# HsinyuG/mobile-manipulator-mpc

Hardware: AMD Instinct MI355X
Metric: MPC solves/sec, whole-body N=20 batch=8192 (higher is better)
Workload: dtype f64

## Files before the change

### __graft_entry__.py

```python
import os
import subprocess
import sys

_ROOT = os.path.dirname(os.path.abspath(__file__))
if _ROOT not in sys.path:
    sys.path.insert(0, _ROOT)


def build():
    import mmpc_loader
    mm = mmpc_loader.load()
    sys.path.insert(0, os.path.join(_ROOT, "tests"))
    import shape_helper
    mm_build = sys.modules[mm.__name__ + ".build"]
    mm_build.build_many(shape_helper.SHAPE_LIST, force=bool(os.environ.get("MMPC_FORCE_BUILD")), jobs=16)
    lib = mm_build.LIB
    assert os.path.exists(lib)
    mm._capi.lib()
    subprocess.check_call(["make", "-s", "-C", os.path.join(_ROOT, "oracle"), "all"])
    shape_helper.build_all(jobs=16)
    shape_helper.wrong_tag_library(mm)
    import emu_helper
    import prim_helper
    import tick_emu_helper
    import mission_emu_helper
    import motion_helper
    import scaling_helper
    emu_helper.build()
    scaling_helper.build()
    motion_helper.build()
    motion_helper.build(asan=True)
    tick_emu_helper.build()
    mission_emu_helper.build()
    for defs in ((), ("MMPC_RCP_NEWTON=1",), ("MMPC_PIV_NEWTON=0",)):
        prim_helper.build(defs)


def smoke():
    import numpy as np
    import mmpc_loader
    from oracle import synth, coracle, nlp
    mm = mmpc_loader.load()
    B = 8
    d = synth.make_batch(B)
    robot = mm.MobileManipulator(0.1)
    ctrl = mm.MPCWholeBody(robot, [], [], N=20, max_batch=B, n_obstacles=5)
    r = ctrl.solve_batch(d["x_init"], d["traj_ref"], d["u_ref"], d["obs"])
    par = nlp.WholeBodyParams()
    o = coracle.solve_batch(par, d["x_init"], d["traj_ref"], d["u_ref"], np.zeros((B, 20, 5)), d["obs"])
    assert (r["status"] == 0).all(), r["status"]
    dX = np.abs(r["X"] - o["X"]).max()
    dU = np.abs(r["U"] - o["U"]).max()
    assert dX < 1e-6 and dU < 1e-6, (dX, dU)
    print("smoke ok: B=%d iters=%s max|dX|=%.2e max|dU|=%.2e" % (B, r["iters"].tolist(), dX, dU))


if __name__ == "__main__":
    build()
    if len(sys.argv) > 1 and sys.argv[1] == "smoke":
        smoke()
```

### mobile-manipulator-mpc_amd/csrc/mmpc_fast.h

```cpp
#pragma once
#include "mmpc_core.h"

#if defined(MMPC_STAMP) && !defined(MMPC_EMU)
__device__ unsigned long long mmpc_stamp_acc[16];
#define MMPC_T0() unsigned long long t_prev_ = __builtin_readcyclecounter(), t_now_, t_acc_[14] = {0, 0, 0, 0, 0, 0, 0, 0, 0, 0, 0, 0, 0, 0};
#define MMPC_TS(i) { t_now_ = __builtin_readcyclecounter(); t_acc_[i] += t_now_ - t_prev_; t_prev_ = t_now_; }
#define MMPC_TEND() { if (threadIdx.x == 0) for (int i_ = 0; i_ < 14; i_++) atomicAdd(&mmpc_stamp_acc[i_], t_acc_[i_]); }
#ifdef MMPC_STAMP_COARSE
#define MMPC_TSF(i)
#else
#define MMPC_TSF(i) MMPC_TS(i)
#endif
#else
#define MMPC_T0()
#define MMPC_TS(i)
#define MMPC_TSF(i)
#define MMPC_TEND()
#endif
#define MMPC_MC_MAX 8

#ifdef MMPC_EMU
MMPC_DEV double mmpc_vmax(double a, double b) { return a > b ? a : b; }
MMPC_DEV double mmpc_vmin(double a, double b) { return a < b ? a : b; }
#else
// ... 3 lines not shown
MMPC_DEV double mmpc_z_safeguard_fast(double z, double t, double mu) {
    const double rt = mmpc_rcp(t);
    return mmpc_vmin(mmpc_vmax(z, (mu * (1.0 / MMPC_KAPPA_SIGMA)) * rt), (MMPC_KAPPA_SIGMA * mu) * rt);
}
MMPC_DEV double mmpc_log_mant(double m, int *ex) {
    int e;
    m = frexp(m, &e);
    if (m < 0.70710678118654752440) { m *= 2.0; e -= 1; }
    *ex += e;
    const double s = (m - 1.0) * mmpc_rcp(m + 1.0), z = s * s;
    double p = 1.0 / 21.0;
    p = fma(p, z, 1.0 / 19.0); p = fma(p, z, 1.0 / 17.0); p = fma(p, z, 1.0 / 15.0); p = fma(p, z, 1.0 / 13.0);
    p = fma(p, z, 1.0 / 11.0); p = fma(p, z, 1.0 / 9.0); p = fma(p, z, 1.0 / 7.0); p = fma(p, z, 1.0 / 5.0);
    p = fma(p, z, 1.0 / 3.0); p = fma(p, z, 1.0);
    return 2.0 * s * p;
}
MMPC_DEV void mmpc_arm_segments_fast(double q1, double q2, double q3, double dr[3], double dz[3]) { mmpc_arm_segments(q1, q2, q3, dr, dz); }
MMPC_HD constexpr int mmpc_y(int a) { return a < 3 ? a : a + 3; }

#ifndef MMPC_UNROLL_NMAX
#define MMPC_UNROLL_NMAX 30
#endif
#ifndef MMPC_FWD_UNROLL
#define MMPC_FWD_UNROLL 64
#endif
#ifndef MMPC_RIC_UNROLL
#define MMPC_RIC_UNROLL 2
#endif
#define MMPC_B(x, q) (((x) >> (8 * (q))) & 255u)
MMPC_DEV double mmpc_box_t(double d) { return mmpc_vmax(d, 1e-15); }

#ifndef MMPC_SAFEGUARD_LAZY
#define MMPC_SAFEGUARD_LAZY 1
#endif
#ifndef MMPC_LEG_DET
#define MMPC_LEG_DET 1
#endif
#ifndef MMPC_D2_ONE_RCP
#define MMPC_D2_ONE_RCP 1
#endif
#ifndef MMPC_PADMAP
#define MMPC_PADMAP 1
#endif
#ifndef MMPC_SLIM_NMIN
#define MMPC_SLIM_NMIN 21
#endif
#ifndef MMPC_RG_NMIN
#define MMPC_RG_NMIN MMPC_SLIM_NMIN
#endif
#ifndef MMPC_RG_MAX
#define MMPC_RG_MAX 3
#endif
template <int KIND, int N>
struct MmpcFastDims {
    typedef MmpcDims<KIND> D;
    static constexpr int NX = D::NX, NU = D::NU, NV = D::NV, NXX = D::NXX, NUU = D::NUU, NSELF = D::NSELF;
    static constexpr int NS = N + 1;
    static constexpr int NPAIR = NS * NV;
    static constexpr bool PADMAP = MMPC_PADMAP && N < MMPC_SLIM_NMIN && NV < 16 && NX <= N && (N * 16 + MMPC_WAVE - 1) / MMPC_WAVE <= (NPAIR + MMPC_WAVE - 1) / MMPC_WAVE;
    static constexpr int TRGS = N >= MMPC_SLIM_NMIN ? 8 : 9;
    static constexpr int NPASS = PADMAP ? (N * 16 + MMPC_WAVE - 1) / MMPC_WAVE : (NPAIR + MMPC_WAVE - 1) / MMPC_WAVE;
    static constexpr int NKB = (NX + 1 + 3) / 4;
    static constexpr int NPU = NU * (NU - 1) / 2;
    static constexpr bool PAIRS = ((NX + 1) & 1) == 0;
    static constexpr int NLEG = PAIRS ? (NU + 1) / 2 : NU;
    static constexpr int RG = ((N >= MMPC_RG_NMIN || KIND == 1) && 2 * NS <= MMPC_WAVE) ? (MMPC_WAVE / NS < MMPC_RG_MAX ? MMPC_WAVE / NS : MMPC_RG_MAX) : 1;
// ... 34 lines not shown
    MmpcFastLayout L{};
    int o = 0;
#define MMPC_CARVE(name, n) L.name = o; o += (n); o = (o + 1) & ~1;
    MMPC_CARVE(XU, F::NS * F::NV) MMPC_CARVE(S, F::NS) MMPC_CARVE(LAM, F::NS * F::NX)
    MMPC_CARVE(XUREF, SLIM ? 0 : F::NS * F::NV) MMPC_CARVE(ULAST, SLIM ? 0 : F::NS * F::NU)
    MMPC_CARVE(OBS, obs_per_stage == 2 ? M * 5 + 1 : (obs_per_stage ? (SLIM ? 0 : F::NS * M * 3) : M * 3))
    MMPC_CARVE(CST, MMPC_C_SIZE) MMPC_CARVE(CV, F::NS * MMPC_NCV) MMPC_CARVE(CD, F::NS * F::NX) MMPC_CARVE(TRG, F::NS * F::TRGS)
    MMPC_CARVE(HXX, F::NS * F::NXX) MMPC_CARVE(QXU, F::NS * F::NV) MMPC_CARVE(HUXL, F::NU * F::NX)
    MMPC_CARVE(HUUL, F::NUU) MMPC_CARVE(HUX02, F::NS) MMPC_CARVE(HUUD, F::NS * F::NU) MMPC_CARVE(SN, 16)
    MMPC_CARVE(KK, GK ? 0 : N * F::NU * (F::NX + 1)) MMPC_CARVE(KF, 0) MMPC_CARVE(DXU, F::NS * F::NV) MMPC_CARVE(DS, F::NS)
    MMPC_CARVE(DLAM, F::NS * F::NX) MMPC_CARVE(RB, F::NS * F::NV) MMPC_CARVE(RDS, F::NS) MMPC_CARVE(Q1V, F::NV + 2) MMPC_CARVE(FILT, 2 * MMPC_FCAP)
    if (GK || F::NS * F::NV >= N * F::NPU) L.KU = L.DXU; else { MMPC_CARVE(KU, N * F::NPU) }
    if (F::NS * F::NX >= MMPC_WAVE) L.DUMP = L.DLAM; else { MMPC_CARVE(DUMP, MMPC_WAVE) } MMPC_CARVE(MISC, 8)
#undef MMPC_CARVE
    L.total = o;
    return L;
}

#define MMPC_NSCAL 12
template <int KIND, int N>
MMPC_HD int mmpc_fast_state_doubles(int MC) {
    typedef MmpcFastDims<KIND, N> F;
    return F::NPAIR + F::NS + F::NS * F::NX + 2 * MMPC_FCAP + MMPC_NSCAL + MMPC_WAVE * (2 * F::NPASS + 2 * (MC > 0 ? MC : 1) + 8);
}

template <int KIND, int N>
struct MmpcFastEnvelope {
    typedef MmpcFastDims<KIND, N> F;
    typedef MmpcGainBlock<KIND, N> GB;
    static constexpr bool SLIM = N >= MMPC_SLIM_NMIN;
    static constexpr bool ROOMY = KIND == 0 && N <= MMPC_UNROLL_NMAX;
    static constexpr int RIC_UNROLL = ROOMY ? MMPC_RIC_UNROLL : 1, FWD_UNROLL = (ROOMY || GB::ON) ? (MMPC_FWD_UNROLL < N ? MMPC_FWD_UNROLL : N) : 1;
    static constexpr int GRS = F::NU * F::NX + F::NU;
    static constexpr bool RING_FITS = !GB::ON || 4 * GRS <= F::NU * F::NX + F::NUU + F::NS + F::NS * F::NU;
    static constexpr bool RING_UNROLLED = !GB::ON || FWD_UNROLL >= N;
    static constexpr bool SLIM_MAP_OK = !(SLIM && F::PADMAP);
    static constexpr bool Q1_ITEMS_OK = F::NXX + F::NU * F::NX + F::NUU + F::NV <= 2 * MMPC_WAVE && F::NV + 2 <= 32;
    static constexpr bool ROLL_ROW_OK = F::NX <= 16;
    static constexpr int nrs(int MC) { return (MC > 0 ? MC : 0) + F::NSELF; }
    static constexpr int soc_used(int MC) { return (F::NS * F::NV + F::NS + F::NS * F::NX) + F::NS * F::NX + F::NS * nrs(MC) + F::NS * F::NX + F::NS * nrs(MC); }
    static constexpr bool soc_ok(int MC) { return soc_used(MC) <= mmpc_soc_doubles(N, F::NX, F::NU, nrs(MC)); }
    static constexpr int mcr(int MC) { return MC > 0 ? (MC + F::RG - 1) / F::RG : 1; }
    static constexpr int LOGF_BOX = 2 * F::NPASS;
    static constexpr int logf_row(int MC) { return (F::RG > 1 ? mcr(MC) : MC) + F::NSELF; }
    static constexpr int logf(int MC) { return LOGF_BOX > logf_row(MC) ? LOGF_BOX : logf_row(MC); }
    static constexpr bool log_high_ok(int MC) { return 19 * logf(MC) < 300; }
    static constexpr bool LOG_LOW_OK = 15 * LOGF_BOX < 300;
    static constexpr bool lds_ok(int MC) {
        for (int ops = 0; ops < 3; ops++) if (mmpc_fast_layout<KIND, N>(MC, ops).total * (int)sizeof(double) > 64 * 1024) return false;
        return true;
    }
    static constexpr bool ok(int MC) {
        return MC >= 0 && F::TILE_OK && SLIM_MAP_OK && Q1_ITEMS_OK && ROLL_ROW_OK && RING_FITS && RING_UNROLLED && LOG_LOW_OK && log_high_ok(MC) &&
               soc_ok(MC) && lds_ok(MC);
    }
};
#define MMPC_SHAPE_NMAX 63
#define MMPC_SHAPE_MMAX 16
template <int KIND, int N = MMPC_SHAPE_NMAX>
struct MmpcEnvelopeScan {
    static constexpr bool ok(int n, int MC) { return n == N ? MmpcFastEnvelope<KIND, N>::ok(MC) : MmpcEnvelopeScan<KIND, N - 1>::ok(n, MC); }
};
template <int KIND>
struct MmpcEnvelopeScan<KIND, 0> { static constexpr bool ok(int, int) { return false; } };
MMPC_HD constexpr bool mmpc_fast_shape_ok(int kind, int N, int M) {
    if (N < 1 || N > MMPC_SHAPE_NMAX || M < 0 || M > MMPC_SHAPE_MMAX) return false;
    return kind == 0 ? MmpcEnvelopeScan<0>::ok(N, M) : (kind == 1 ? MmpcEnvelopeScan<1>::ok(N, M) : false);
}

template <int KIND, int N, int MC>
struct MmpcLaneState {
    typedef MmpcFastDims<KIND, N> F;
    double lo_z[F::NPASS], hi_z[F::NPASS];
    double b_lo[F::NPASS], b_hi[F::NPASS];
    static constexpr int MCR = MmpcFastEnvelope<KIND, N>::mcr(MC);
    double ct[MCR], cz[MCR], cdt[MCR];
    double cp[F::RG > 1 ? 9 : 1];
    double st[4], sz[4], sdt[4];
    double hss, gss, vx[6];
    unsigned ab_o[F::NKB];
    unsigned h_o[4], h_l[4];
    unsigned h_m;
    unsigned p_o[4];
    int kl_b[F::NLEG], kl_s[F::NLEG];
    MmpcAcc rP, rT, rM;
    double rAB[F::NKB], opa, opb;
    double mg[4], pv0, pv1;
    double nab[F::NKB], nhm[4];
    unsigned f_v, f_x;
    unsigned q1d[2];
    double fw[MMPC_FW_SLOTS];
    int fw_a[5];
};

#ifndef MMPC_EMU
MMPC_DEV double mmpc_op_add(double a, double b) { return a + b; }
MMPC_WAVE_RED(mmpc_wave_sum, mmpc_op_add)
MMPC_WAVE_RED(mmpc_wave_max, mmpc_vmax)
MMPC_WAVE_RED(mmpc_wave_min, mmpc_vmin)
MMPC_WAVE_RED4(mmpc_wave_sum4, mmpc_op_add)
MMPC_WAVE_RED4(mmpc_wave_max4, mmpc_vmax)
#define MMPC_RED4_SUM(i0, i1, i2, i3, out) mmpc_wave_sum4(wr_one[i0], wr_one[i1], wr_one[i2], wr_one[i3], out)
#define MMPC_RED4_MAX(i0, i1, i2, i3, out) mmpc_wave_max4(wr_one[i0], wr_one[i1], wr_one[i2], wr_one[i3], out)
#define MMPC_RED_SUM(i) mmpc_wave_sum(wr_one[i])
#define MMPC_RED_MAX(i) mmpc_wave_max(wr_one[i])
#define MMPC_RED_MIN(i) mmpc_wave_min(wr_one[i])
#else
static inline double mmpc_emu_red(double (*wr)[9], int i, int op) {
    double v[MMPC_WAVE], w[MMPC_WAVE];
    for (int l = 0; l < MMPC_WAVE; l++) v[l] = wr[l][i];
    for (int q = 0; q < 6; q++) {
        const int o = 1 << q;
// ... 364 lines not shown

    int status = 1, it = 0, nfilt = 0, filt_init = 0;
    double E0 = 0.0, th_max = 0.0, th_min = 0.0;
    int nsmall_r = 0;
    double prox_r = 0.0, delta_r = 0.0, dprev_r = 0.0;
    if (CONT && io.resume) {
        const double *const st_xu = io.state, *const st_s = io.state + ST_S, *const st_lam = io.state + ST_LAM,
                     *const st_filt = io.state + ST_FILT, *const st_scal = io.state + ST_SCAL, *const st_lane = io.state + ST_LANE;
        LANES_BEGIN
        auto &ls = MMPC_LS;
        for (int i = lane; i < NPAIR; i += MMPC_WAVE) XU[i] = st_xu[i];
        for (int i = lane; i < NS; i += MMPC_WAVE) S[i] = st_s[i];
        for (int i = lane; i < NS * NX; i += MMPC_WAVE) LAM[i] = st_lam[i];
        for (int i = lane; i < 2 * MMPC_FCAP; i += MMPC_WAVE) FILT[i] = st_filt[i];
        const double *q = st_lane + lane * NLREG;
#pragma unroll
        for (int p = 0; p < NPASS; p++) { ls.lo_z[p] = q[p]; ls.hi_z[p] = q[NPASS + p]; }
#pragma unroll
        for (int m = 0; m < MCR; m++) { ls.ct[m] = q[2 * NPASS + m]; ls.cz[m] = q[2 * NPASS + MCS + m]; }
#pragma unroll
        for (int i = 0; i < 4; i++) { ls.st[i] = q[2 * NPASS + 2 * MCS + i]; ls.sz[i] = q[2 * NPASS + 2 * MCS + 4 + i]; }
        LANES_END
        mu = st_scal[0]; th_max = st_scal[1]; th_min = st_scal[2]; prox_r = st_scal[3];
        it = (int)st_scal[4]; nfilt = (int)st_scal[5]; filt_init = (int)st_scal[6]; nsmall_r = (int)st_scal[7]; delta_r = st_scal[8]; dprev_r = st_scal[9];
    }
    const int it_start = CONT ? it : 0;
    double err_d = 0.0, err_p = 0.0, tzmax = 0.0, tzmin = 0.0, zsum = 0.0, cost_c = 0.0, th_c = 0.0, sumlog = 0.0;
    int in_ls = 0, lspass = 0, lsi = 0, nsmall = nsmall_r;
    double prox = prox_r;
    double delta_last = delta_r;
    double delta_prev = dprev_r;
    double alpha = 0.0, ap = 1.0, ad = 1.0, dphi = 0.0, phi0 = 0.0, th0 = 0.0;

    auto apply_step = [&](double d_alpha, bool first) {
        double pz_lo = 1e300, pz_hi = 0.0;
        auto zsafe = [&](double zn, double tn) -> double {
            if (!MMPC_SAFEGUARD_LAZY) return mmpc_z_safeguard_fast(zn, tn, mu);
            const double pz = zn * tn;
            pz_lo = mmpc_vmin(pz_lo, pz); pz_hi = mmpc_vmax(pz_hi, pz);
            return zn;
        };
        LANES_BEGIN
        auto &ls = MMPC_LS;
        {
            MMPC_ROW_LANE
            if (rlane) {
#pragma unroll
                for (int r = 0; r < MCR; r++) {
                    if (RG == 1 || rs + RG * r < M) {
                        const double t = ls.ct[r], z = ls.cz[r], dtv = ls.cdt[r], tn = t + d_alpha * dtv;
                        if (first) { const double it_ = mmpc_rcp(t); ls.cz[r] = zsafe(z + ad * (mu * it_ - z - z * it_ * dtv), tn); }
                        ls.ct[r] = tn;
                    }
                }
            }
        }
        if (lane < NS) {
#pragma unroll
            for (int i = 0; i < NSELF; i++) {
                const double t = ls.st[i], z = ls.sz[i], dtv = ls.sdt[i], tn = t + d_alpha * dtv;
                if (first) { const double it_ = mmpc_rcp(t); ls.sz[i] = zsafe(z + ad * (mu * it_ - z - z * it_ * dtv), tn); }
                ls.st[i] = tn;
            }
        }
        MMPC_PAIR_SETUP
#pragma unroll
        for (int p = 0; p < NPASS; p++) {
            MMPC_PAIR(p)
            if (pok) {
                const double val = XU[idx], dv = DXU[idx], vn = val + d_alpha * dv;
                if (first) {
                    const double lo = ls.b_lo[p], hi = ls.b_hi[p];
                    const bool alo = lo > -1e299, ahi = hi < 1e299;
                    if (alo) { const double z = ls.lo_z[p], it_ = mmpc_rcp(mmpc_box_t(val - lo)); ls.lo_z[p] = zsafe(z + ad * (mu * it_ - z - z * it_ * dv), mmpc_box_t(vn - lo)); }
                    if (ahi) { const double z = ls.hi_z[p], it_ = mmpc_rcp(mmpc_box_t(hi - val)); ls.hi_z[p] = zsafe(z + ad * (mu * it_ - z + z * it_ * dv), mmpc_box_t(hi - vn)); }
                }
                if (idx >= NX) XU[idx] = vn;
            }
        }
        for (int i = lane; i < NS * NX; i += MMPC_WAVE) if (i >= NX) LAM[i] += d_alpha * DLAM[i];
        for (int i = lane; i < NS; i += MMPC_WAVE) S[i] += d_alpha * DS[i];
        LANES_END
#ifdef MMPC_SAFEGUARD_FORCE
        constexpr bool zforce = true;
#else
        constexpr bool zforce = false;
#endif
        if (MMPC_SAFEGUARD_LAZY && first && MMPC_WAVE_ANY(zforce || !(pz_lo >= 2.0 * mu * (1.0 / MMPC_KAPPA_SIGMA) && pz_hi <= 0.5 * MMPC_KAPPA_SIGMA * mu))) {
            LANES_BEGIN
            auto &ls = MMPC_LS;
            {
                MMPC_ROW_LANE
                if (rlane) {
#pragma unroll
                    for (int r = 0; r < MCR; r++) if (RG == 1 || rs + RG * r < M) ls.cz[r] = mmpc_z_safeguard_fast(ls.cz[r], ls.ct[r], mu);
                }
            }
            if (lane < NS) {
#pragma unroll
                for (int i = 0; i < NSELF; i++) ls.sz[i] = mmpc_z_safeguard_fast(ls.sz[i], ls.st[i], mu);
            }
            MMPC_PAIR_SETUP
#pragma unroll
            for (int p = 0; p < NPASS; p++) {
                MMPC_PAIR(p)
                if (pok) {
                    const double lo = ls.b_lo[p], hi = ls.b_hi[p], vn = XU[idx];
                    if (lo > -1e299) ls.lo_z[p] = mmpc_z_safeguard_fast(ls.lo_z[p], mmpc_box_t(vn - lo), mu);
                    if (hi < 1e299) ls.hi_z[p] = mmpc_z_safeguard_fast(ls.hi_z[p], mmpc_box_t(hi - vn), mu);
                }
            }
            LANES_END
        }
    };

    constexpr int NRS = (MC > 0 ? MC : 0) + NSELF;
    constexpr int O_D = 0, O_TC = O_D + NS * NV + NS + NS * NX, O_TR = O_TC + NS * NX,
                  O_AC = O_TR + NS * NRS, O_AR = O_AC + NS * NX;
    static_assert(O_AR + NS * NRS == ENV::soc_used(MC) && ENV::soc_ok(MC), "second-order correction scratch");
    int soc_st = 0, soc_p = 0, fatal = 0;
    double a_soc = 0.0, alpha0 = 0.0, a_prev = 0.0, th_prev = 0.0;
#ifdef MMPC_EMU
#define MMPC_SOC_FENCE()
#else
#define MMPC_SOC_FENCE() { __builtin_amdgcn_fence(__ATOMIC_RELEASE, "workgroup"); __builtin_amdgcn_fence(__ATOMIC_ACQUIRE, "workgroup"); }
#endif
    auto soc_dir = [&](bool save) {
        LANES_BEGIN
        double *q = io.soc + O_D;
        for (int i = lane; i < NS * NV; i += MMPC_WAVE) { if (save) q[i] = DXU[i]; else DXU[i] = q[i]; }
        for (int i = lane; i < NS; i += MMPC_WAVE) { if (save) q[NS * NV + i] = DS[i]; else DS[i] = q[NS * NV + i]; }
        for (int i = lane; i < NS * NX; i += MMPC_WAVE) { if (save) q[NS * NV + NS + i] = DLAM[i]; else DLAM[i] = q[NS * NV + NS + i]; }
        LANES_END
        MMPC_SOC_FENCE()
    };
    auto soc_rows = [&](bool acc, bool first) {
        LANES_BEGIN
        auto &ls = MMPC_LS;
        double *tc = io.soc + O_TC, *tr = io.soc + O_TR, *ac = io.soc + O_AC, *ar = io.soc + O_AR;
        for (int i = lane; i < N * NX; i += MMPC_WAVE) {
            if (!acc) tc[i] = CD[i];
            else { const double v = a_prev * (first ? CD[i] : ac[i]) + tc[i]; ac[i] = v; CD[i] = v; }
        }
        {
            MMPC_ROW_LANE
            if (rlane && (RG > 1 || lane < NS)) {
// ... 85 lines not shown
```

### mobile-manipulator-mpc_amd/csrc/mmpc_fast_d2.inc

```
        LANES_BEGIN
        auto &ls = MMPC_LS;
        double rp = 0.0, rd = 0.0, dphi = 0.0;
#undef MMPC_D2_ROW
#if MMPC_D2_ONE_RCP
#define MMPC_D2_ROW(t, z, dtv) { const double r_ = mmpc_rcp((t) * (z)), a_ = (dtv) * (r_ * (z));                                  \
            rp = mmpc_vmax(rp, -a_); rd = mmpc_vmax(rd, (1.0 + a_) - mu * r_); dphi -= mu * a_; }
#else
#define MMPC_D2_ROW(t, z, dtv) { const double it_ = mmpc_rcp(t), dzv_ = mu * it_ - (z) - (z) * it_ * (dtv);                        \
            rp = mmpc_vmax(rp, -(dtv) * it_); rd = mmpc_vmax(rd, -dzv_ * mmpc_rcp(z)); dphi -= mu * (dtv) * it_; }
#endif
        if (RG > 1 && M > 0) {
            MMPC_ROW_LANE
            if (rlane) {
                const double dx0 = DXU[MMPC_MUL24(rk, NV)], dx1 = DXU[MMPC_MUL24(rk, NV) + 1], dsk = DS[rk];
                const double px = XU[MMPC_MUL24(rk, NV)], py = XU[MMPC_MUL24(rk, NV) + 1], sk = S[rk];
                double ob[MCR * 3];
#pragma unroll
                for (int r = 0; r < MCR; r++) {
                    const MmpcObs o = obs_ptr(rk, rs + RG * r < M ? rs + RG * r : 0);
                    ob[3 * r] = o.x(); ob[3 * r + 1] = o.y(); ob[3 * r + 2] = o.r();
                }
#pragma unroll
                for (int r = 0; r < MCR; r++) {
                    if (rs + RG * r < M) {
                        const double ddx = px - ob[3 * r], ddy = py - ob[3 * r + 1], m2 = ddx * ddx + ddy * ddy, id = mmpc_rsqrt(m2), d = m2 * id;
                        const double hv = (ob[3 * r + 2] + MMPC_BASE_R) - d - sk;
                        const double t = ls.ct[r], z = ls.cz[r];
                        const double jd = -(ddx * dx0 + ddy * dx1) * id - dsk;
                        double res = hv + t;
                        if constexpr (socm) res = io.soc[O_AR + rk * NRS + rs + RG * r];
                        const double dtv = -res - jd;
                        ls.cdt[r] = dtv;
                        MMPC_D2_ROW(t, z, dtv)
                    }
                }
            }
        }
        if (lane < NS) {
            const int k = lane;
            const double *dx = DXU + MMPC_MUL24(k, NV);
            const double dsk = DS[k], dsks = DS[slack_idx(k)];
            const double px = XU[MMPC_MUL24(k, NV)], py = XU[MMPC_MUL24(k, NV) + 1], sk = S[k];
            double ob[(MC > 0 ? MC : 1) * 3];
#pragma unroll
            for (int m = 0; m < (RG > 1 ? 0 : M); m++) { const MmpcObs o = obs_ptr(k, m); ob[3 * m] = o.x(); ob[3 * m + 1] = o.y(); ob[3 * m + 2] = o.r(); }
#pragma unroll
            for (int m = 0; m < (RG > 1 ? 0 : M); m++) {
                const double ddx = px - ob[3 * m], ddy = py - ob[3 * m + 1], m2 = ddx * ddx + ddy * ddy, id = mmpc_rsqrt(m2), d = m2 * id;
                const double hv = (ob[3 * m + 2] + MMPC_BASE_R) - d - sk;
                const double t = ls.ct[m], z = ls.cz[m];
                const double jd = -(ddx * dx[0] + ddy * dx[1]) * id - dsk;
                double res = hv + t;
                if constexpr (socm) res = io.soc[O_AR + k * NRS + m];
                const double dtv = -res - jd;
                ls.cdt[m] = dtv;
                MMPC_D2_ROW(t, z, dtv)
            }
            double sn = 0.0, cs = 0.0, dr[3] = {0, 0, 0}, dz[3] = {0, 0, 0};
            if (NSELF) {
                sn = TRG[MMPC_MUL24(k, F::TRGS)]; cs = TRG[MMPC_MUL24(k, F::TRGS) + 1];
#pragma unroll
                for (int a = 0; a < 3; a++) { dr[a] = TRG[MMPC_MUL24(k, F::TRGS) + 2 + a]; dz[a] = TRG[MMPC_MUL24(k, F::TRGS) + 5 + a]; }
            }
            const double sks = S[slack_idx(k)];
#pragma unroll
            for (int i = 0; i < NSELF; i++) {
                double g6[6];
                const double hv = mmpc_self_row(i, px, py, cs, sn, dr, dz, g6) - sks;
                const double t = ls.st[i], z = ls.sz[i];
                double jd = -dsks;
#pragma unroll
                for (int a = 0; a < 6; a++) jd += g6[a] * dx[mmpc_y(a)];
                double res = hv + t;
                if constexpr (socm) res = io.soc[O_AR + k * NRS + M + i];
                const double dtv = -res - jd;
                ls.sdt[i] = dtv;
                MMPC_D2_ROW(t, z, dtv)
            }
            dphi += 2 * Sw * S[k] * dsk;
        }
        MMPC_PAIR_SETUP
#pragma unroll
        for (int p = 0; p < NPASS; p++) {
            MMPC_PAIR(p)
            if (pok) {
                const double lo = ls.b_lo[p], hi = ls.b_hi[p];
                const bool alo = lo > -1e299, ahi = hi < 1e299;
                const double val = XU[idx], dv = DXU[idx];
                dphi += RB[idx] * dv;
                if (alo) {
                    const double t = mmpc_box_t(val - lo), z = ls.lo_z[p], dtv = dv;
                    MMPC_D2_ROW(t, z, dtv)
                }
                if (ahi) {
                    const double t = mmpc_box_t(hi - val), z = ls.hi_z[p], dtv = -dv;
                    MMPC_D2_ROW(t, z, dtv)
                }
            }
        }
        MMPC_WR(0) = rp; MMPC_WR(1) = rd; MMPC_WR(2) = dphi;
        LANES_END
```

### mobile-manipulator-mpc_amd/csrc/mmpc_fast_iter.inc

```
        MMPC_TS(0)
        if (RG > 1 && M > 0) {
            LANES_BEGIN
            auto &ls = MMPC_LS;
            double e_p = 0.0, tzmax = 0.0, tzmin = 1e300, zsum = 0.0, th = 0.0, rb0 = 0.0, rb1 = 0.0, rz = 0.0;
            MmpcLogAcc la; la.init();
            MMPC_ROW_LANE
            if (rlane) {
                const double px = XU[MMPC_MUL24(rk, NV)], py = XU[MMPC_MUL24(rk, NV) + 1], sk = S[rk];
                double ob[MCR * 3];
#pragma unroll
                for (int r = 0; r < MCR; r++) {
                    const MmpcObs o = obs_ptr(rk, rs + RG * r < M ? rs + RG * r : 0);
                    ob[3 * r] = o.x(); ob[3 * r + 1] = o.y(); ob[3 * r + 2] = o.r();
                }
#pragma unroll
                for (int r = 0; r < MCR; r++) {
                    if (rs + RG * r < M) {
                        const double dx = px - ob[3 * r], dy = py - ob[3 * r + 1], m2 = dx * dx + dy * dy, id = mmpc_rsqrt(m2), d = m2 * id;
                        const double nxv = dx * id, nyv = dy * id;
                        const double h = (ob[3 * r + 2] + MMPC_BASE_R) - d - sk;
                        const double t = ls.ct[r], z = ls.cz[r];
                        rb0 -= nxv * z; rb1 -= nyv * z; rz += z;
                        e_p = mmpc_vmax(e_p, fabs(h + t)); th += fabs(h + t); la.mul(t);
                        tzmax = mmpc_vmax(tzmax, t * z); tzmin = mmpc_vmin(tzmin, t * z); zsum += z;
// ... 189 lines not shown
#else
            const double a_t = alpha;
#endif
            const bool ftype = dphi < 0 && th0 <= th_min && a_t * mmpc_powf(-dphi, 2.3f) > mmpc_powf(th0, 1.1f);
            bool accepted = false, augment = false;
            if (okf) {
                if (ftype) accepted = phi <= phi0 + 1e-8 * a_t * dphi + 1e-14 * fabs(phi0);
                else if (th <= (1 - 1e-5) * th0 || phi <= phi0 - 1e-5 * th0) { accepted = true; augment = true; }
            }
            if (augment) {
                int slot = nfilt;
                if (nfilt >= MMPC_FCAP) { slot = 0; for (int i = 1; i < MMPC_FCAP; i++) if (FILT[2 * i] > FILT[2 * slot]) slot = i; }
                else nfilt++;
                LANES_BEGIN
                if (lane == 0) { FILT[2 * slot] = (1 - 1e-5) * th0; FILT[2 * slot + 1] = phi0 - 1e-5 * th0; }
                LANES_END
            }
#if MMPC_ITER_SOC
            if (soc_st == 2) {
                if (accepted) { soc_st = 0; alpha = a_soc; }
                else if (th > 0.99 * th_prev || soc_p + 1 >= MMPC_SOC_MAX) {
                    apply_step(-a_soc, false);
                    soc_dir(false);
                    soc_st = 3; in_ls = 0;
                    continue;
                } else {
                    soc_rows(false, false);
                    apply_step(-a_soc, false);
                    soc_p++; a_prev = a_soc; th_prev = th; soc_st = 1; in_ls = 0;
                    continue;
                }
            }
#else
            if (__builtin_expect(!accepted && MMPC_SOC_MAX > 0 && lsi == 0 && lspass == 0 && io.soc && th >= th0 && th0 <= th_min, 0)) {
                th_prev = th; soc_enter = true;
                break;
            }
#endif
            if (!accepted) {
                double anext = alpha;
                bool retry = false;
                if (lsi < MMPC_MAX_LS - 1) { anext = 0.5 * alpha; lsi++; retry = true; }
                else if (lspass == 0 && nfilt > 0) { nfilt = 0; lspass = 1; lsi = 0; anext = ap; retry = true; }
                if (retry) { apply_step(anext - alpha, false); alpha = anext; continue; }
            }
            in_ls = 0;
            mmpc_prox_update(ap, alpha, prox, nsmall);
            MMPC_TS(12)
#if MMPC_ITER_SOC
            break;
#endif
        }
#if MMPC_ITER_SOC
        if (soc_st == 1) soc_rows(true, soc_p == 0);
#else
        {
        double sd = (zsum + zeq_c) * inv_rows, sc = zsum * inv_nrows;
        sd = (sd > 100.0 ? sd : 100.0) * 0.01;
        sc = (sc > 100.0 ? sc : 100.0) * 0.01;
        const double isd = mmpc_rcp(sd), isc = mmpc_rcp(sc);
        E0 = mmpc_vmax(mmpc_vmax(err_d * isd, err_p), tzmax * isc);
        if (!mmpc_finite(E0) || !mmpc_finite(th_c + cost_c + zsum + zeq_c)) {
#ifdef MMPC_EMU_DEBUG
            fprintf(stderr, "E0 nan it %d: err_d %g err_p %g tzmax %g tzmin %g zsum %g sumlog %g\n", it, err_d, err_p, tzmax, tzmin, zsum, sumlog);
#endif
            status = 2; MMPC_ITER_LEAVE }
        if (E0 <= tol) { status = 0; MMPC_ITER_LEAVE }
// ... 11 lines not shown
#pragma unroll
            for (int p = 0; p < NPASS; p++) { q[p] = ls.lo_z[p]; q[NPASS + p] = ls.hi_z[p]; }
#pragma unroll
            for (int m = 0; m < MCR; m++) { q[2 * NPASS + m] = ls.ct[m]; q[2 * NPASS + MCS + m] = ls.cz[m]; }
#pragma unroll
            for (int i = 0; i < 4; i++) { q[2 * NPASS + 2 * MCS + i] = ls.st[i]; q[2 * NPASS + 2 * MCS + 4 + i] = ls.sz[i]; }
            if (lane == 0) {
                st_scal[0] = mu; st_scal[1] = th_max; st_scal[2] = th_min; st_scal[3] = prox;
                st_scal[4] = (double)it; st_scal[5] = (double)nfilt; st_scal[6] = (double)filt_init; st_scal[7] = (double)nsmall; st_scal[8] = delta_last; st_scal[9] = delta_prev;
                st_scal[10] = CST[MMPC_C_SCALE];
            }
            LANES_END
            status = 3;
            MMPC_ITER_LEAVE
        }
        {
            bool changed = false;
            for (;;) {
                const double compmu = mmpc_vmax(fabs(tzmax - mu), fabs(tzmin - mu));
                const double Emu = mmpc_vmax(mmpc_vmax(err_d * isd, err_p), compmu * isc);
                if (!(Emu <= 10.0 * mu && mu > tol / 10)) break;
                mu = mmpc_vmax(tol / 10, mmpc_vmin(0.2 * mu, mu * sqrt(mu)));
                changed = true;
            }
            if (changed) filt_init = 0;
        }
        phi0 = cost_c - mu * sumlog;
        th0 = th_c;
        }
#endif

        MMPC_TS(2)
        int failed = 0;
        double dw = delta_prev > MMPC_IC_SKIP0 ? mmpc_vmax(1e-20, MMPC_IC_DN * delta_last) : 0.0;
#if MMPC_ITER_SOC
        if (soc_st != 3)
#endif
        {
#pragma unroll 1
        for (;;) {
            const bool exact = P.max_iter >= 0;
            constexpr bool dyn_curv = true;
            const double reg = prox + dw;
            int ric_bad = 0;
            {
            constexpr bool socm = MMPC_ITER_SOC != 0; (void)socm;
#include "mmpc_fast_a1r.inc"
            }
            {
            constexpr bool socm = MMPC_ITER_SOC != 0; (void)socm;
#include "mmpc_fast_a1s.inc"
            }
            if (NSELF) {
                LANES_BEGIN
                auto &ls = MMPC_LS;
                const double nih = -Q1V[NV + 1];
#pragma unroll
                for (int t = 0; t < 2; t++) {
                    const unsigned d = ls.q1d[t];
                    double *dst = lds + (d >> 12);
                    const double a = Q1V[d & 31u], b = Q1V[(d >> 5) & 31u], old = *dst;
                    const double base = (d & 1024u) ? old : 0.0;
                    *dst = (d & 2048u) ? fma(a, b, base) : fma(nih, a * b, base);
                }
                LANES_END
            }
// ... 96 lines not shown
                    }
                    LANES_END_REG
                    MMPC_MFMA(rM, ls.opa, ls.opb)
                    if (leg == 0) { MMPC_NEXT_OPERANDS }
                    LANES_BEGIN_NL
                    auto &ls = MMPC_LS;
                    if (!(ls.pv0 > 0.0 && ls.pv1 > 0.0)) ric_bad = 1;
                    *(double *)((char *)KBASE + (unsigned)(ls.kl_b[leg] + MMPC_MUL24(k, ls.kl_s[leg]))) = ls.opa;
                    LANES_END_REG
                }
#undef MMPC_NEXT_OPERANDS
                MMPC_TSF(7)
                LANES_BEGIN_NL
                auto &ls = MMPC_LS;
#pragma unroll
                for (int r = 0; r < 4; r++) {
                    ls.rP[r] = ls.rM[r];
                    const unsigned o = ls.p_o[r];
                    lds[(o & 0xffffu) + k * (int)(o >> 16)] = ls.rM[r];
                    ls.rM[r] = ls.nhm[r];
                }
#pragma unroll
                for (int r = 0; r < NKB; r++) ls.rAB[r] = ls.nab[r];
                LANES_END
            }
            if (ric_bad) failed = 1;
            if (!failed) {
                if (dw > 0.0) delta_last = dw;
#if !MMPC_ITER_SOC
                delta_prev = dw;
#endif
                break;
            }
            dw = dw == 0.0 ? (delta_last == 0.0 ? MMPC_IC_D0 : mmpc_vmax(1e-20, MMPC_IC_DN * delta_last)) : MMPC_IC_UP * dw;
            if (dw > 1e40) break;
            failed = 0;
        }
        if (failed) {
#ifdef MMPC_EMU_DEBUG
            fprintf(stderr, "riccati failed twice it %d\n", it);
#endif
            status = 2; fatal = 1; }
        if (!fatal) {
        LANES_BEGIN
        if constexpr (!GK && NX + 1 <= 16) {
            const int g = lane >> 4, c = lane & 15;
            const bool col = c <= NX;
            constexpr int NTRIP = (N + 3) / 4;
            const int kb = MMPC_MUL24(g, NU * KS) + (col ? c : 0), ub = MMPC_MUL24(g, NPU);
            double kv[NTRIP][NU], cu[NTRIP][NPU > 0 ? NPU : 1];
#pragma unroll
            for (int t = 0; t < NTRIP; t++) {
                const bool in = 4 * (t + 1) <= N || 4 * t + g < N;
                const int kt = in ? kb + t * 4 * NU * KS : 0, ut = in ? ub + t * 4 * NPU : 0;
#pragma unroll
                for (int a = 0; a < NU; a++) kv[t][a] = KK[kt + a * KS];
#pragma unroll
                for (int q = 0; q < NPU; q++) cu[t][q] = KU[ut + q];
            }
#pragma unroll
            for (int t = 0; t < NTRIP; t++) {
#pragma unroll
                for (int a = NU - 1; a >= 0; a--) {
                    double v = kv[t][a];
#pragma unroll
                    for (int b2 = a + 1; b2 < NU; b2++) v += cu[t][a * (2 * NU - a - 1) / 2 + (b2 - a - 1)] * kv[t][b2];
// ... 139 lines not shown
                double dx[NX];
#ifndef MMPC_EMU
                static_assert(ENV::ROLL_ROW_OK, "the roll-out's row lanes must share a row of 16 lanes");
                mmpc_rowbcast_all<0, NX>(ls.fw[MMPC_FW_SLOT(k)], dx);
#else
#pragma unroll
                for (int j = 0; j < NX; j++) dx[j] = MMPC_LANE_GET(fw[MMPC_FW_SLOT(k)], j);
#endif
                double d0 = kf0, d1 = 0.0, d2 = 0.0;
#pragma unroll
                for (int j = 0; j < NX; j += 3) {
                    d0 += kr[j] * dx[j];
                    if (j + 1 < NX) d1 += kr[j + 1] * dx[j + 1];
                    if (j + 2 < NX) d2 += kr[j + 2] * dx[j + 2];
                }
                double v = c0 + ls.fw[MMPC_FW_SLOT(k)];
                double w = cf[0] * dx[2];
                v += cf[1] * dx[3];
                w += cf[2] * dx[4];
                v += cf[3] * dx[5];
                const double du = d0 + (d1 + d2);
                v = (v + w) + cf[4] * du;
                ls.fw[MMPC_FW_SLOT(k + 1)] = v;
                lds[fw_du + k * fw_st] = du;
                lds[fw_dx + k * fw_st] = v;
                LANES_END_REG
            }
            LANES_BEGIN
            LANES_END
        }
        MMPC_TS(9)
        LANES_BEGIN
        auto &ls = MMPC_LS;
        if (lane < NS) {
            const int k = lane;
            double dx[NX], pk[NXX], y[NX];
#pragma unroll
            for (int j = 0; j < NX; j++) { dx[j] = DXU[MMPC_MUL24(k, NV) + j]; y[j] = QXU[MMPC_MUL24(k, NV) + j] + LAM[MMPC_MUL24(k, NX) + j]; }
#pragma unroll
            for (int e = 0; e < NXX; e++) pk[e] = HXX[MMPC_MUL24(k, NXX) + e];
#pragma unroll
            for (int i = 0; i < NX; i++) {
#pragma unroll
                for (int j = 0; j < NX; j++) y[i] += pk[i >= j ? i * (i + 1) / 2 + j : j * (j + 1) / 2 + i] * dx[j];
            }
#pragma unroll
            for (int i = 0; i < NX; i++) DLAM[MMPC_MUL24(k, NX) + i] = -y[i];
            double vdx = 0.0;
            constexpr int ny = NSELF ? 6 : 2;
#pragma unroll
            for (int a = 0; a < ny; a++) vdx += ls.vx[a] * dx[mmpc_y(a)];
            if (k == N - 1 && NSELF) {
#pragma unroll
                for (int a = 0; a < 6; a++) vdx += SN[4 + a] * DXU[N * NV + mmpc_y(a)];
            }
            DS[k] = -(ls.gss - vdx) * mmpc_rcp(ls.hss);
            if (k == N) { for (int c = 0; c < NU; c++) DXU[N * NV + NX + c] = 0.0; }
        }
        LANES_END
        }
        }
        if (fatal) MMPC_ITER_LEAVE
        MMPC_TS(10)
        const double tau = mmpc_vmax(0.99, 1.0 - mu);
#if MMPC_ITER_SOC
        if (soc_st == 1) {
        constexpr bool socm = true; (void)socm;
#include "mmpc_fast_d2.inc"
        } else
#endif
        {
        constexpr bool socm = false; (void)socm;
#include "mmpc_fast_d2.inc"
        }
        {
            double r4[4];
            MMPC_RED4_MAX(0, 1, 0, 1, r4);
            const double rp_ = r4[0], rd_ = r4[1], ap_n = rp_ > tau ? tau * mmpc_rcp(rp_) : 1.0;
#if MMPC_ITER_SOC
            if (soc_st == 1) {
                a_soc = ap_n;
                apply_step(a_soc, false);
                soc_st = 2; in_ls = 1;
                continue;
            }
#endif
            ap = ap_n; ad = rd_ > tau ? tau * mmpc_rcp(rd_) : 1.0; dphi = MMPC_RED_SUM(2);
#if MMPC_ITER_SOC
            if (soc_st == 3) {
                alpha = 0.5 * ap; lsi = 1; lspass = 0;
                apply_step(alpha, false);
                soc_st = 0; in_ls = 1;
                continue;
            }
#endif
        }

#if !MMPC_ITER_SOC
        MMPC_TS(11)
        if (!filt_init) { nfilt = 0; th_max = 1e4 * mmpc_vmax(1.0, th0); th_min = 1e-4 * mmpc_vmax(1.0, th0); filt_init = 1; }
        alpha = ap; lspass = 0; lsi = 0;
        apply_step(alpha, true);
        in_ls = 1;
        it++;
#endif
```

Before: 1.438 million.

## Fuse first step application with direction pass using register-cached step deltas

Caches the per-lane step quantities computed in the fraction-to-boundary pass (dual step deltas, box values, step directions, slack and state deltas) in lane registers. A new finish_step then applies the first full step from these registers instead of re-reading the shared-memory arrays and recomputing the dual updates in apply_step. The intent is to cut LDS traffic and repeated arithmetic on each Newton iteration, in exchange for more per-lane register state, which may lower occupancy or cause spills. Dead-value markers let the compiler drop these registers outside their live range.

After: 1.445 million, median of 6. No clear change (+0.5%).

```diff
diff --git a/__graft_entry__.py b/__graft_entry__.py
--- a/__graft_entry__.py
+++ b/__graft_entry__.py
@@ -26,8 +26,10 @@
     import mission_emu_helper
     import motion_helper
     import scaling_helper
+    import step_helper
     emu_helper.build()
     scaling_helper.build()
+    step_helper.build(("MMPC_STEP_FUSED=1",))
     motion_helper.build()
     motion_helper.build(asan=True)
     tick_emu_helper.build()
diff --git a/mobile-manipulator-mpc_amd/csrc/mmpc_fast.h b/mobile-manipulator-mpc_amd/csrc/mmpc_fast.h
--- a/mobile-manipulator-mpc_amd/csrc/mmpc_fast.h
+++ b/mobile-manipulator-mpc_amd/csrc/mmpc_fast.h
@@ -59,6 +59,20 @@
 
 #ifndef MMPC_SAFEGUARD_LAZY
 #define MMPC_SAFEGUARD_LAZY 1
+#endif
+#ifndef MMPC_STEP_FUSED
+#define MMPC_STEP_FUSED 1
+#endif
+#if defined(MMPC_EMU) && defined(MMPC_EMU_COUNTERS)
+static thread_local long mmpc_emu_counters[4];
+#define MMPC_COUNT(i) { mmpc_emu_counters[i]++; }
+#else
+#define MMPC_COUNT(i) {}
+#endif
+#ifdef MMPC_EMU
+#define MMPC_DEAD(x) { (x) = NAN; }
+#else
+#define MMPC_DEAD(x) { (x) = __builtin_nondeterministic_value(x); }
 #endif
 #ifndef MMPC_LEG_DET
 #define MMPC_LEG_DET 1
@@ -159,6 +173,7 @@
     static constexpr bool ROOMY = KIND == 0 && N <= MMPC_UNROLL_NMAX;
     static constexpr int RIC_UNROLL = ROOMY ? MMPC_RIC_UNROLL : 1, FWD_UNROLL = (ROOMY || GB::ON) ? (MMPC_FWD_UNROLL < N ? MMPC_FWD_UNROLL : N) : 1;
     static constexpr int GRS = F::NU * F::NX + F::NU;
+    static constexpr bool STEP_FUSED = MMPC_STEP_FUSED != 0;
     static constexpr bool RING_FITS = !GB::ON || 4 * GRS <= F::NU * F::NX + F::NUU + F::NS + F::NS * F::NU;
     static constexpr bool RING_UNROLLED = !GB::ON || FWD_UNROLL >= N;
     static constexpr bool SLIM_MAP_OK = !(SLIM && F::PADMAP);
@@ -205,6 +220,9 @@
     double cp[F::RG > 1 ? 9 : 1];
     double st[4], sz[4], sdt[4];
     double hss, gss, vx[6];
+    double d_ds, d_dx[6];
+    double cdz[MCR], sdz[4];
+    double pval[F::NPASS], pdv[F::NPASS], pdzl[F::NPASS], pdzh[F::NPASS];
     unsigned ab_o[F::NKB];
     unsigned h_o[4], h_l[4];
     unsigned h_m;
@@ -635,6 +653,38 @@
     double delta_prev = dprev_r;
     double alpha = 0.0, ap = 1.0, ad = 1.0, dphi = 0.0, phi0 = 0.0, th0 = 0.0;
 
+#ifdef MMPC_SAFEGUARD_FORCE
+    constexpr bool zforce = true;
+#else
+    constexpr bool zforce = false;
+#endif
+    auto exact_clamp = [&]() {
+        MMPC_COUNT(2)
+        LANES_BEGIN
+        auto &ls = MMPC_LS;
+        {
+            MMPC_ROW_LANE
+            if (rlane) {
+#pragma unroll
+                for (int r = 0; r < MCR; r++) if (RG == 1 || rs + RG * r < M) ls.cz[r] = mmpc_z_safeguard_fast(ls.cz[r], ls.ct[r], mu);
+            }
+        }
+        if (lane < NS) {
+#pragma unroll
+            for (int i = 0; i < NSELF; i++) ls.sz[i] = mmpc_z_safeguard_fast(ls.sz[i], ls.st[i], mu);
+        }
+        MMPC_PAIR_SETUP
+#pragma unroll
+        for (int p = 0; p < NPASS; p++) {
+            MMPC_PAIR(p)
+            if (pok) {
+                const double lo = ls.b_lo[p], hi = ls.b_hi[p], vn = XU[idx];
+                if (lo > -1e299) ls.lo_z[p] = mmpc_z_safeguard_fast(ls.lo_z[p], mmpc_box_t(vn - lo), mu);
+                if (hi < 1e299) ls.hi_z[p] = mmpc_z_safeguard_fast(ls.hi_z[p], mmpc_box_t(hi - vn), mu);
+            }
+        }
+        LANES_END
+    };
     auto apply_step = [&](double d_alpha, bool first) {
         double pz_lo = 1e300, pz_hi = 0.0;
         auto zsafe = [&](double zn, double tn) -> double {
@@ -684,37 +734,55 @@
         for (int i = lane; i < NS * NX; i += MMPC_WAVE) if (i >= NX) LAM[i] += d_alpha * DLAM[i];
         for (int i = lane; i < NS; i += MMPC_WAVE) S[i] += d_alpha * DS[i];
         LANES_END
-#ifdef MMPC_SAFEGUARD_FORCE
-        constexpr bool zforce = true;
-#else
-        constexpr bool zforce = false;
-#endif
-        if (MMPC_SAFEGUARD_LAZY && first && MMPC_WAVE_ANY(zforce || !(pz_lo >= 2.0 * mu * (1.0 / MMPC_KAPPA_SIGMA) && pz_hi <= 0.5 * MMPC_KAPPA_SIGMA * mu))) {
-            LANES_BEGIN
-            auto &ls = MMPC_LS;
-            {
-                MMPC_ROW_LANE
-                if (rlane) {
-#pragma unroll
-                    for (int r = 0; r < MCR; r++) if (RG == 1 || rs + RG * r < M) ls.cz[r] = mmpc_z_safeguard_fast(ls.cz[r], ls.ct[r], mu);
+        if (MMPC_SAFEGUARD_LAZY && first && MMPC_WAVE_ANY(zforce || !(pz_lo >= 2.0 * mu * (1.0 / MMPC_KAPPA_SIGMA) && pz_hi <= 0.5 * MMPC_KAPPA_SIGMA * mu))) exact_clamp();
+    };
+    auto finish_step = [&](double a_p) {
+        double pz_lo = 1e300, pz_hi = 0.0;
+        auto zsafe = [&](double zn, double tn) -> double {
+            if (!MMPC_SAFEGUARD_LAZY) return mmpc_z_safeguard_fast(zn, tn, mu);
+            const double pz = zn * tn;
+            pz_lo = mmpc_vmin(pz_lo, pz); pz_hi = mmpc_vmax(pz_hi, pz);
+            return zn;
+        };
+        LANES_BEGIN
+        auto &ls = MMPC_LS;
+        {
+            MMPC_ROW_LANE
+            if (rlane) {
+#pragma unroll
+                for (int r = 0; r < MCR; r++) {
+                    if (RG == 1 || rs + RG * r < M) {
+                        const double tn = ls.ct[r] + a_p * ls.cdt[r];
+                        ls.cz[r] = zsafe(ls.cz[r] + ad * ls.cdz[r], tn);
+                        ls.ct[r] = tn;
+                    }
                 }
             }
-            if (lane < NS) {
-#pragma unroll
-                for (int i = 0; i < NSELF; i++) ls.sz[i] = mmpc_z_safeguard_fast(ls.sz[i], ls.st[i], mu);
-            }
-            MMPC_PAIR_SETUP
-#pragma unroll
-            for (int p = 0; p < NPASS; p++) {
-                MMPC_PAIR(p)
-                if (pok) {
-                    const double lo = ls.b_lo[p], hi = ls.b_hi[p], vn = XU[idx];
-                    if (lo > -1e299) ls.lo_z[p] = mmpc_z_safeguard_fast(ls.lo_z[p], mmpc_box_t(vn - lo), mu);
-                    if (hi < 1e299) ls.hi_z[p] = mmpc_z_safeguard_fast(ls.hi_z[p], mmpc_box_t(hi - vn), mu);
-                }
-            }
-            LANES_END
-        }
+        }
+        if (lane < NS) {
+#pragma unroll
+            for (int i = 0; i < NSELF; i++) {
+                const double tn = ls.st[i] + a_p * ls.sdt[i];
+                ls.sz[i] = zsafe(ls.sz[i] + ad * ls.sdz[i], tn);
+                ls.st[i] = tn;
+            }
+        }
+        MMPC_PAIR_SETUP
+#pragma unroll
+        for (int p = 0; p < NPASS; p++) {
+            MMPC_PAIR(p)
+            if (pok) {
+                const double vn = ls.pval[p] + a_p * ls.pdv[p];
+                const double lo = ls.b_lo[p], hi = ls.b_hi[p];
+                if (lo > -1e299) ls.lo_z[p] = zsafe(ls.lo_z[p] + ad * ls.pdzl[p], mmpc_box_t(vn - lo));
+                if (hi < 1e299) ls.hi_z[p] = zsafe(ls.hi_z[p] + ad * ls.pdzh[p], mmpc_box_t(hi - vn));
+                if (idx >= NX) XU[idx] = vn;
+            }
+        }
+        for (int i = lane; i < NS * NX; i += MMPC_WAVE) if (i >= NX) LAM[i] += a_p * DLAM[i];
+        for (int i = lane; i < NS; i += MMPC_WAVE) S[i] += a_p * DS[i];
+        LANES_END
+        if (MMPC_SAFEGUARD_LAZY && MMPC_WAVE_ANY(zforce || !(pz_lo >= 2.0 * mu * (1.0 / MMPC_KAPPA_SIGMA) && pz_hi <= 0.5 * MMPC_KAPPA_SIGMA * mu))) exact_clamp();
     };
 
     constexpr int NRS = (MC > 0 ? MC : 0) + NSELF;
diff --git a/mobile-manipulator-mpc_amd/csrc/mmpc_fast_d2.inc b/mobile-manipulator-mpc_amd/csrc/mmpc_fast_d2.inc
--- a/mobile-manipulator-mpc_amd/csrc/mmpc_fast_d2.inc
+++ b/mobile-manipulator-mpc_amd/csrc/mmpc_fast_d2.inc
@@ -1,6 +1,14 @@
         LANES_BEGIN
         auto &ls = MMPC_LS;
         double rp = 0.0, rd = 0.0, dphi = 0.0;
+        if constexpr (fused) {
+#pragma unroll
+            for (int r = 0; r < MCR; r++) MMPC_DEAD(ls.cdz[r])
+#pragma unroll
+            for (int i = 0; i < 4; i++) MMPC_DEAD(ls.sdz[i])
+#pragma unroll
+            for (int p = 0; p < NPASS; p++) { MMPC_DEAD(ls.pval[p]) MMPC_DEAD(ls.pdv[p]) MMPC_DEAD(ls.pdzl[p]) MMPC_DEAD(ls.pdzh[p]) }
+        }
 #undef MMPC_D2_ROW
 #if MMPC_D2_ONE_RCP
 #define MMPC_D2_ROW(t, z, dtv) { const double r_ = mmpc_rcp((t) * (z)), a_ = (dtv) * (r_ * (z));                                  \
@@ -9,6 +17,10 @@
 #define MMPC_D2_ROW(t, z, dtv) { const double it_ = mmpc_rcp(t), dzv_ = mu * it_ - (z) - (z) * it_ * (dtv);                        \
             rp = mmpc_vmax(rp, -(dtv) * it_); rd = mmpc_vmax(rd, -dzv_ * mmpc_rcp(z)); dphi -= mu * (dtv) * it_; }
 #endif
+#undef MMPC_D2_KEEP
+#define MMPC_D2_KEEP(dst, t, z, dtv) if constexpr (fused) { const double it_ = mmpc_rcp(t); dst = mu * it_ - (z) - (z) * it_ * (dtv); }
+#undef MMPC_D2_DX
+#define MMPC_D2_DX(a) (fused ? ls.d_dx[a] : dx[mmpc_y(a)])
         if (RG > 1 && M > 0) {
             MMPC_ROW_LANE
             if (rlane) {
@@ -31,15 +43,17 @@
                         if constexpr (socm) res = io.soc[O_AR + rk * NRS + rs + RG * r];
                         const double dtv = -res - jd;
                         ls.cdt[r] = dtv;
+                        MMPC_D2_KEEP(ls.cdz[r], t, z, dtv)
                         MMPC_D2_ROW(t, z, dtv)
                     }
                 }
             }
         }
+        const double ds_n1 = fused ? MMPC_LANE_GET(d_ds, N - 1) : 0.0;
         if (lane < NS) {
             const int k = lane;
-            const double *dx = DXU + MMPC_MUL24(k, NV);
-            const double dsk = DS[k], dsks = DS[slack_idx(k)];
+            const double *dx = DXU + MMPC_MUL24(k, NV); (void)dx;
+            const double dsk = fused ? ls.d_ds : DS[k], dsks = fused ? (k < N ? ls.d_ds : ds_n1) : DS[slack_idx(k)];
             const double px = XU[MMPC_MUL24(k, NV)], py = XU[MMPC_MUL24(k, NV) + 1], sk = S[k];
             double ob[(MC > 0 ? MC : 1) * 3];
 #pragma unroll
@@ -49,11 +63,12 @@
                 const double ddx = px - ob[3 * m], ddy = py - ob[3 * m + 1], m2 = ddx * ddx + ddy * ddy, id = mmpc_rsqrt(m2), d = m2 * id;
                 const double hv = (ob[3 * m + 2] + MMPC_BASE_R) - d - sk;
                 const double t = ls.ct[m], z = ls.cz[m];
-                const double jd = -(ddx * dx[0] + ddy * dx[1]) * id - dsk;
+                const double jd = -(ddx * MMPC_D2_DX(0) + ddy * MMPC_D2_DX(1)) * id - dsk;
                 double res = hv + t;
                 if constexpr (socm) res = io.soc[O_AR + k * NRS + m];
                 const double dtv = -res - jd;
                 ls.cdt[m] = dtv;
+                MMPC_D2_KEEP(ls.cdz[m], t, z, dtv)
                 MMPC_D2_ROW(t, z, dtv)
             }
             double sn = 0.0, cs = 0.0, dr[3] = {0, 0, 0}, dz[3] = {0, 0, 0};
@@ -70,11 +85,12 @@
                 const double t = ls.st[i], z = ls.sz[i];
                 double jd = -dsks;
 #pragma unroll
-                for (int a = 0; a < 6; a++) jd += g6[a] * dx[mmpc_y(a)];
+                for (int a = 0; a < 6; a++) jd += g6[a] * MMPC_D2_DX(a);
                 double res = hv + t;
                 if constexpr (socm) res = io.soc[O_AR + k * NRS + M + i];
                 const double dtv = -res - jd;
                 ls.sdt[i] = dtv;
+                MMPC_D2_KEEP(ls.sdz[i], t, z, dtv)
                 MMPC_D2_ROW(t, z, dtv)
             }
             dphi += 2 * Sw * S[k] * dsk;
@@ -88,12 +104,15 @@
                 const bool alo = lo > -1e299, ahi = hi < 1e299;
                 const double val = XU[idx], dv = DXU[idx];
                 dphi += RB[idx] * dv;
+                if constexpr (fused) { ls.pval[p] = val; ls.pdv[p] = dv; }
                 if (alo) {
                     const double t = mmpc_box_t(val - lo), z = ls.lo_z[p], dtv = dv;
+                    MMPC_D2_KEEP(ls.pdzl[p], t, z, dv)
                     MMPC_D2_ROW(t, z, dtv)
                 }
                 if (ahi) {
                     const double t = mmpc_box_t(hi - val), z = ls.hi_z[p], dtv = -dv;
+                    if constexpr (fused) { const double it_ = mmpc_rcp(t); ls.pdzh[p] = mu * it_ - z + z * it_ * dv; }
                     MMPC_D2_ROW(t, z, dtv)
                 }
             }
diff --git a/mobile-manipulator-mpc_amd/csrc/mmpc_fast_iter.inc b/mobile-manipulator-mpc_amd/csrc/mmpc_fast_iter.inc
--- a/mobile-manipulator-mpc_amd/csrc/mmpc_fast_iter.inc
+++ b/mobile-manipulator-mpc_amd/csrc/mmpc_fast_iter.inc
@@ -245,7 +245,9 @@
                 }
             }
 #else
+            if (!accepted && lsi == 0 && lspass == 0) MMPC_COUNT(0)
             if (__builtin_expect(!accepted && MMPC_SOC_MAX > 0 && lsi == 0 && lspass == 0 && io.soc && th >= th0 && th0 <= th_min, 0)) {
+                MMPC_COUNT(1)
                 th_prev = th; soc_enter = true;
                 break;
             }
@@ -323,6 +325,7 @@
 
         MMPC_TS(2)
         int failed = 0;
+        constexpr bool fused = ENV::STEP_FUSED && !MMPC_ITER_SOC; (void)fused;
         double dw = delta_prev > MMPC_IC_SKIP0 ? mmpc_vmax(1e-20, MMPC_IC_DN * delta_last) : 0.0;
 #if MMPC_ITER_SOC
         if (soc_st != 3)
@@ -485,6 +488,7 @@
 #endif
                 break;
             }
+            MMPC_COUNT(3)
             dw = dw == 0.0 ? (delta_last == 0.0 ? MMPC_IC_D0 : mmpc_vmax(1e-20, MMPC_IC_DN * delta_last)) : MMPC_IC_UP * dw;
             if (dw > 1e40) break;
             failed = 0;
@@ -690,6 +694,11 @@
         MMPC_TS(9)
         LANES_BEGIN
         auto &ls = MMPC_LS;
+        if constexpr (fused) {
+            MMPC_DEAD(ls.d_ds)
+#pragma unroll
+            for (int a = 0; a < 6; a++) MMPC_DEAD(ls.d_dx[a])
+        }
         if (lane < NS) {
             const int k = lane;
             double dx[NX], pk[NXX], y[NX];
@@ -712,7 +721,13 @@
 #pragma unroll
                 for (int a = 0; a < 6; a++) vdx += SN[4 + a] * DXU[N * NV + mmpc_y(a)];
             }
-            DS[k] = -(ls.gss - vdx) * mmpc_rcp(ls.hss);
+            const double dsv = -(ls.gss - vdx) * mmpc_rcp(ls.hss);
+            DS[k] = dsv;
+            if constexpr (fused) {
+                ls.d_ds = dsv;
+#pragma unroll
+                for (int a = 0; a < ny; a++) ls.d_dx[a] = dx[mmpc_y(a)];
+            }
             if (k == N) { for (int c = 0; c < NU; c++) DXU[N * NV + NX + c] = 0.0; }
         }
         LANES_END
@@ -758,7 +773,7 @@
         MMPC_TS(11)
         if (!filt_init) { nfilt = 0; th_max = 1e4 * mmpc_vmax(1.0, th0); th_min = 1e-4 * mmpc_vmax(1.0, th0); filt_init = 1; }
         alpha = ap; lspass = 0; lsi = 0;
-        apply_step(alpha, true);
+        if constexpr (fused) finish_step(alpha); else apply_step(alpha, true);
         in_ls = 1;
         it++;
 #endif
```
